# bio-phys/BioEM

Measured on AMD Instinct MI355X. Metric: image-comparisons/sec (orient×CTF×particle) at 224²; log P max-abs-diff vs CPU, higher is better.
Workload: dtype f32

## Files before the change

### bioem_amd/csrc/bioem_hip.hip

```cpp
#define BIOEM_MAIN_TU 1
#include "engine_types.hpp"

#include <rccl/rccl.h>

#include <dlfcn.h>

#include <map>
#include <memory>
#include <mutex>
#include <queue>
#include <string>
#include <vector>

namespace
{

struct HipErr
{
  std::string msg;
};

#define HIP_CHECK(h, expr)                                                                                         \
  do                                                                                                               \
  {                                                                                                                \
// ... 1119 lines not shown
    const int Rl = 2 * P.halfR, off = fastm2_off(Rl, P.gs), nAcc = fastm2_acc(Rl, P.gs);
    const int nS = (P.N1 + 1) / 2;
    twk.assign((size_t) nS * nAcc * 2, make_float2(0.f, 0.f));
    for (int s2 = 0; s2 < nS; s2++)
      for (int ac = 0; ac < nAcc; ac++)
      {
        const long long dx = (long long) (2 * off * (ac / off) + (ac % off) - kFm2WD) * P.gs;
        for (int e = 0; e < 2; e++)
          if (2 * s2 + e < P.N1)
            twk[((size_t) s2 * nAcc + ac) * 2 + e] = twiddle(dx * (2 * s2 + e), N);
      }
    std::vector<float> bt(fastm2_btab_floats(h->H, P.nyq));
    for (size_t K = 0; K < bt.size() / 192; K++)
      for (int ct = 0; ct < 3; ct++)
        for (int l = 0; l < 64; l++)
        {
          const long long ky = 2 * (long long) K + (l >> 5), dy = (long long) (16 * ct + (l & 15) - kFm2WD) * P.gs;
          const float2 w = twiddle(ky * dy, N);
          bt[(K * 3 + ct) * 64 + l] = ((l >> 4) & 1) ? w.y : w.x;
        }
    if (upload(h, h->dBtab, bt.data(), bt.size()))
      return 1;
  }
  if (P.family == KF_FAST || P.family == KF_FASTM || P.family == KF_ROWS || P.family == KF_ODDFFT)
  {
    const int NW = 2 * P.winD + 1;
    const int nK1 = P.family == KF_ROWS ? N : P.N1;
    twk.resize((size_t) nK1 * NW);
    for (int k1 = 0; k1 < nK1; k1++)
      for (int d = -P.winD; d <= P.winD; d++)
        twk[(size_t) k1 * NW + d + P.winD] = twiddle((long long) d * P.gs * k1, N);
  }
  if (!twk.empty() && upload(h, h->dTwk, twk.data(), twk.size()))
    return 1;
  if (P.nyq)
  {
    const int NW = 2 * P.nyqWD + 1, R2 = P.halfR;
    std::vector<float2> twn((size_t) (N / 2) * NW * 2);
    for (int k1 = 0; k1 < P.N1; k1++)
      for (int k2p = 0; k2p < R2; k2p++)
        for (int m = -P.nyqWD; m <= P.nyqWD; m++)
          for (int e = 0; e < 2; e++)
          {
            const long long kx = (long long) P.N1 * (2 * k2p + e) + k1;
            twn[(((size_t) (k1 * R2 + k2p) * NW) + (m + P.nyqWD)) * 2 + e] = twiddle(kx * m * P.gs, N);
          }
    if (upload(h, h->dTwNyq, twn.data(), twn.size()))
      return 1;
  }
  std::vector<float2> tw(N + 1);
  std::vector<double2> twd(N);
  for (int k = 0; k <= N; k++)
    tw[k] = twiddle(k, N);
  for (int k = 0; k < N; k++)
    twd[k] = twiddle_d(k, N);
  std::vector<double2> lt(64);
  for (int i = 0; i < 64; i++)
  {
    const double c = 1.0 / (1.0 + ((double) i + 0.5) / 64.0);
    lt[i] = make_double2(c, -log(c));
  }
  if (upload(h, h->dTw, tw.data(), tw.size()) || upload(h, h->dTwD, twd.data(), twd.size()) ||
      upload(h, h->dDisp, P.disp.data(), P.disp.size()) || upload(h, h->dLtab, lt.data(), lt.size()))
    return 1;
  if (const char *lg = getenv("BIOEM_SIGNATURE_LOG"))
    if (FILE *f = fopen(lg, "a"))
    {
      fprintf(f, "%s\n", bioem_hip_kernel_signature(h));
      if (P.nyq)
        fprintf(f, "k_nyquist_rows<%d, %d>\n", P.nyqWD, h->nMaps <= 64 ? 4 : 1);
      fclose(f);
    }
  return 0;
}

int bioem_hip_create(bioem_hip_handle *out, int device, const bioem_hip_param_device *pd, int nMaps, int nAngles,
                     int nCTF, int algo)
{
  return create_impl(out, device, pd, nMaps, nAngles, nCTF, algo, false, 0, nAngles);
}

int bioem_hip_create_shard(bioem_hip_handle *out, int device, const bioem_hip_param_device *pd, int nMaps, int nAngles,
                           int nCTF, int algo, int iOrientBegin, int iOrientEnd)
{
  return create_impl(out, device, pd, nMaps, nAngles, nCTF, algo, true, iOrientBegin, iOrientEnd);
}

int bioem_hip_destroy(bioem_hip_handle h)
{
  if (!h)
    return 0;
  hipSetDevice(h->device);
  if (h->stream)
    hipStreamSynchronize(h->stream);
  drain_events(h);
  drain_phases(h);
  for (hipEvent_t e : h->evPool)
    hipEventDestroy(e);
  if (h->prepStream)
    hipStreamSynchronize(h->prepStream);
  for (const bioem_hip_ctx::Alloc &al : h->allocs)
    if (al.pinned)
      hipHostFree(al.p);
    else
      hipFree(al.p);
  for (int k = 0; k < 2; k++)
// ... 1130 lines not shown
```

### bioem_amd/csrc/compare_args.hpp

```cpp
#ifndef BIOEM_COMPARE_ARGS_HPP
#define BIOEM_COMPARE_ARGS_HPP

namespace
{

struct CompareArgs
{
  const float2 *ref;
  const float2 *conv;
  const bioem_hip_param5 *params;
  const double2 *postc;
  const float *sumRef, *sumsqRef;
  const float2 *tw;
  const int *disp;
  const double2 *ltab;
  const float2 *twk;
  const float2 *twnyq;
  const float *btab;
  float *tnyq;
  Partial *partials;
  int ldPart;
  int N, H, N1, nd, maxD, nOC, nMaps, algo;
  int Hp;
  int pchunk;
  int gs;
  int ndx, ndy;
  int ts, nyqWD;
  int split;
  PD pd;
};

}

#endif
```

### bioem_amd/csrc/compare_fast.hpp

```cpp
#ifndef BIOEM_COMPARE_FAST_HPP
#define BIOEM_COMPARE_FAST_HPP

namespace
{

typedef const float2 __attribute__((address_space(4))) *const_float2_ptr;
__device__ __forceinline__ const_float2_ptr as_constant(const float2 *p)
{
  return (const_float2_ptr) (unsigned long long) p;
}

template <typename T>
__device__ __forceinline__ T *uniform_ptr(T *p)
{
  const unsigned long long v = (unsigned long long) p;
  const unsigned lo = __builtin_amdgcn_readfirstlane((unsigned) v);
  const unsigned hi = __builtin_amdgcn_readfirstlane((unsigned) (v >> 32));
  return (T *) (((unsigned long long) hi << 32) | lo);
}

__device__ __noinline__ double log_slow_path(float f) { return log((double) f); }

__device__ __forceinline__ double log_of_float(float f, const double2 *ltab)
{
// ... 144 lines not shown
  for (int v = 0; v < B; v++)
  {
    double lp = w.A * lg[v] + w.t2;
    lp -= w.prior;
    lpf[v] = ok[v] ? (float) lp : -INFINITY;
    lpe[v] = (algo == 1) ? (double) lpf[v] : lp;
  }
  float mb = lpf[0], vb = cc[0];
  int ib = ok[0] ? id[0] : 0x7fffffff;
#pragma unroll
  for (int v = 1; v < B; v++)
  {
    const bool t = ok[v] && (lpf[v] > mb || (lpf[v] == mb && id[v] < ib));
    mb = t ? lpf[v] : mb;
    ib = t ? id[v] : ib;
    vb = t ? cc[v] : vb;
  }
  const bool take = mb > L.m || (mb == L.m && ib < L.id);
  const float newm = fmaxf(L.m, mb);
  double sum = (L.m == newm) ? L.s : L.s * exp_fast_nonpos((double) L.m - (double) newm);
#pragma unroll
  for (int v = 0; v < B; v++)
  {
    const double e = exp_fast_nonpos(lpe[v] - (double) newm);
    sum += ok[v] ? e : 0.;
  }
  L.s = sum;
  L.m = newm;
  L.id = take ? ib : L.id;
  L.val = take ? vb : L.val;
}

__device__ __forceinline__ bool fast_block_pair(const CompareArgs &a, int &p, int &ocg)
{
  const int ocGroups = (a.nOC + 3) >> 2;
  if (a.pchunk < 0)
  {
    const int x = blockIdx.x & 7, q = blockIdx.x >> 3;
    ocg = (q / a.nMaps) * 8 + x;
    p = q % a.nMaps;
    return ocg < ocGroups;
  }
  const int per = a.pchunk * ocGroups;
  int c = blockIdx.x / per;
  const int nch = (a.nMaps + a.pchunk - 1) / a.pchunk;
  c = min(c, nch - 1);
  const int rem = blockIdx.x - c * per;
  const int pc = min(a.pchunk, a.nMaps - c * a.pchunk);
  ocg = rem / pc;
  p = c * a.pchunk + (rem - ocg * pc);
  return true;
}

template <int NR, bool STATIC, int NP, int TS>
__device__ __forceinline__ void window_accumulate(const float2 *Tl, const float2 *twl, int N, int step, int idx0,
                                                  const int (&rowoff)[NR], int nr, float (&acc)[NR], int npairs = NP)
{
  int idx = idx0;
#pragma unroll 2
  for (int kp = 0; kp < npairs; kp++)
  {
    const float2 w0 = twl[idx];
    idx += step;
    if (idx >= N)
      idx -= N;
    const float2 w1 = twl[idx];
    idx += step;
    if (idx >= N)
      idx -= N;
#pragma unroll
    for (int r = 0; r < NR; r++)
    {
      if (STATIC || r < nr)
      {
        const float4 t = *reinterpret_cast<const float4 *>(&Tl[(STATIC ? rowoff[0] + r * TS : rowoff[r]) + 2 * kp]);
        float v = acc[r];
        v = fmaf(t.x, w0.x, v);
        v = fmaf(-t.y, w0.y, v);
        v = fmaf(t.z, w1.x, v);
        v = fmaf(-t.w, w1.y, v);
        acc[r] = v;
      }
    }
  }
}

#define FFT_IN(k) (is_pow2(R) ? bitrevR<R>(k) : DIGITREV<R>.pos[k])
#define FFT_OUT(n) (n)
#define FFT_RUN(xr, xi)                                                                                            \
  do                                                                                                               \
  {                                                                                                                \
    if constexpr (is_pow2(R))                                                                                      \
      fft_inverse_dit<R>(xr, xi);                                                                                  \
    else                                                                                                           \
      fft_inverse_mixed<R>(xr, xi);                                                                                \
  } while (0)
template <int WD, int R, bool NYQ, int GS>
__global__ __launch_bounds__(256, 3) void k_compare_fast(const CompareArgs a)
{
  static_assert(WD <= 10, "windows of at most 21 rows; 27 / 31 rows: k_compare_fastm");
  constexpr int NW = 2 * WD + 1;
  constexpr int R2 = R / 2;
  constexpr int RD = (R2 % 4 == 0) ? 4 : (R2 == 15) ? 3 : (R2 % 5 == 0) ? 5 : (R2 % 3 == 0) ? 3 : (R2 % 2 == 0) ? 2 : 1;
  constexpr int NR = (WD <= 5) ? 3 : 7;
  constexpr int TS = 66;
  extern __shared__ __align__(16) unsigned char smem[];
  const int N = a.N, H = a.H, N1 = a.N1;
  float2 *twl = reinterpret_cast<float2 *>(smem);
  int *displ = reinterpret_cast<int *>(smem + (size_t) ((N + 2) & ~1) * 8);
  double2 *ltab = reinterpret_cast<double2 *>(smem + (size_t) ((N + 2) & ~1) * 8 + 256);
  float2 *Tall = reinterpret_cast<float2 *>(smem + (size_t) ((N + 2) & ~1) * 8 + 256 + 1024);
  const int wave = __builtin_amdgcn_readfirstlane((int) (threadIdx.x >> 6));
  const int lane = threadIdx.x & 63;
  float2 *Tl = Tall + (size_t) wave * NW * TS;

  for (int t = threadIdx.x; t <= N; t += blockDim.x)
    twl[t] = a.tw[t];
  int *dinv = displ + 32;
  const int mD = a.maxD / GS;
  for (int t = threadIdx.x; t < a.nd; t += blockDim.x)
  {
    const int dv = a.disp[t];
    displ[t] = dv;
    const int m = dv / GS + mD;
    if (m >= 0 && m < 32)
      dinv[m] = t;
  }
  for (int t = threadIdx.x; t < 64; t += blockDim.x)
    ltab[t] = a.ltab[t];
  __syncthreads();

  int p, ocg;
  if (!fast_block_pair(a, p, ocg))
    return;
  const int oc_raw = ocg * 4 + wave;
  const bool oc_valid = oc_raw < a.nOC;
  const int oc = oc_valid ? oc_raw : a.nOC - 1;
  const int Hp = a.Hp;
  const size_t M = (size_t) N * Hp;
  const auto rsrcF = __builtin_amdgcn_make_buffer_rsrc(uniform_ptr(const_cast<float2 *>(a.ref + (size_t) p * M)), 0,
                                                       (int) (M * sizeof(float2)), 0x00020000);
  const auto rsrcC = __builtin_amdgcn_make_buffer_rsrc(uniform_ptr(const_cast<float2 *>(a.conv + (size_t) oc * M)), 0,
                                                       (int) (M * sizeof(float2)), 0x00020000);

  const int nd = a.nd;
  const int G = 64 / nd;
  const int nr = (nd + G - 1) / G;
  const int iy = lane % nd, grp = lane / nd;
  const bool wactive = grp < G;
  const int dy = displ[iy];
  const int step = dy < 0 ? dy + N : dy;
  const bool is_static = (nr == NR) && (nd == G * NR) && (nd == 2 * mD + 1);
  float acc[NR];
#pragma unroll
  for (int r = 0; r < NR; r++)
    acc[r] = 0.f;
  auto row_of = [&](int r) -> int {
    int ix = wactive ? grp * nr + r : r;
    if (ix >= nd)
      ix = nd - 1;
    return (displ[ix] / GS + WD) * TS;
  };
  const int rowbase = is_static ? ((wactive ? grp : 0) * NR - mD + WD) * TS : row_of(0);

  const int nblk = NYQ ? (H - 1 + 63) / 64 : (H + 63) / 64;
  const unsigned rowbytes = (unsigned) Hp * 16u;
  constexpr bool SPLIT_OK = !(NYQ && R == 32);
  const int sHalf = (N1 + 1) >> 1;
  const int hsel = lane >> 5;
  const unsigned halfoff = (unsigned) (hsel * sHalf * R2) * rowbytes;
  auto lane_offset = [&](int b) -> unsigned {
    const bool sp = SPLIT_OK && a.split && b == nblk - 1;
    const int kyb = b * 64 + (sp ? (lane & 31) : lane);
    return (unsigned) (kyb < H ? kyb : H - 1) * 16u + (sp ? halfoff : 0u);
  };
  u32x4 rf[RD], rc[RD];
  {
    const unsigned lo0 = lane_offset(0);
#pragma unroll
    for (int t = 0; t < RD; t++)
    {
      rf[t] = __builtin_amdgcn_raw_buffer_load_b128(rsrcF, lo0, (unsigned) t * rowbytes, 0);
      rc[t] = __builtin_amdgcn_raw_buffer_load_b128(rsrcC, lo0, (unsigned) t * rowbytes, 0);
    }
  }
  for (int blk = 0; blk < nblk; blk++)
  {
    const bool split = SPLIT_OK && a.split && blk == nblk - 1;
    const int n1 = split ? sHalf : N1;
    const int ttotal = R2 * n1;
    const int ky = blk * 64 + (split ? (lane & 31) : lane);
    const unsigned laneoff = lane_offset(blk);
    const unsigned laneoff_next = lane_offset(min(blk + 1, nblk - 1));
    const bool has_next = blk + 1 < nblk;
    float Tr[NW], Ti[NW];
#pragma unroll
    for (int d = 0; d < NW; d++)
    {
      Tr[d] = 0.f;
      Ti[d] = 0.f;
    }
    if (ky < H)
    for (int k1 = 0; k1 < n1; k1++)
    {
      float xr[R], xi[R];
      float2 wk[NW];
      const float2 *twk = a.twk + (size_t) k1 * NW;
#pragma unroll
      for (int d = 0; d < NW; d++)
        wk[d] = twk[d];
#pragma unroll
      for (int k2p = 0; k2p < R2; k2p++)
      {
        const float4 f = as_float4(rf[k2p % RD]);
        const float4 c = as_float4(rc[k2p % RD]);
        xr[FFT_IN(2 * k2p)] = fmaf(c.x, f.x, c.y * f.y);
        xi[FFT_IN(2 * k2p)] = fmaf(c.y, f.x, -(c.x * f.y));
        xr[FFT_IN(2 * k2p + 1)] = fmaf(c.z, f.z, c.w * f.w);
        xi[FFT_IN(2 * k2p + 1)] = fmaf(c.w, f.z, -(c.z * f.w));
        int tn = k1 * R2 + k2p + RD;
        unsigned vo = laneoff;
        if (k2p + RD >= R2 && tn >= ttotal)
        {
          tn = has_next ? tn - ttotal : ttotal - 1;
          vo = has_next ? laneoff_next : laneoff;
        }
        rf[k2p % RD] = __builtin_amdgcn_raw_buffer_load_b128(rsrcF, vo, (unsigned) tn * rowbytes, 0);
        rc[k2p % RD] = __builtin_amdgcn_raw_buffer_load_b128(rsrcC, vo, (unsigned) tn * rowbytes, 0);
        __builtin_amdgcn_sched_barrier(0);
      }
      FFT_RUN(xr, xi);
#pragma unroll
      for (int d = -WD; d <= WD; d++)
      {
        const int pos = FFT_OUT((((d * GS) % R) + R) % R);
        const float2 w = wk[d + WD];
        float tr = Tr[d + WD], ti = Ti[d + WD];
        tr = fmaf(xr[pos], w.x, tr);
        tr = fmaf(-xi[pos], w.y, tr);
        ti = fmaf(xr[pos], w.y, ti);
        ti = fmaf(xi[pos], w.x, ti);
        Tr[d + WD] = tr;
        Ti[d + WD] = ti;
      }
    }
    if (split)
    {
      const float2 *ws = a.twk + (size_t) sHalf * NW;
#pragma unroll
      for (int d = 0; d < NW; d++)
      {
        const float2 w = ws[d];
        const float wx = hsel ? w.x : 1.f, wy = hsel ? w.y : 0.f;
        const float tr = fmaf(-Ti[d], wy, Tr[d] * wx), ti = fmaf(Ti[d], wx, Tr[d] * wy);
        const u32x2 sr = __builtin_amdgcn_permlane32_swap(__float_as_uint(tr), __float_as_uint(tr), false, false);
        const u32x2 si = __builtin_amdgcn_permlane32_swap(__float_as_uint(ti), __float_as_uint(ti), false, false);
        Tr[d] = __uint_as_float(sr.x) + __uint_as_float(sr.y);
        Ti[d] = __uint_as_float(si.x) + __uint_as_float(si.y);
      }
    }
    float wgt = 2.f;
    if (ky == 0 || (((N & 1) == 0) && ky == N / 2))
      wgt = 1.f;
    if (ky >= H || (split && hsel))
      wgt = 0.f;
    {
      __syncthreads();
#pragma unroll
      for (int d = 0; d < NW; d++)
        Tl[d * TS + lane] = make_float2(Tr[d] * wgt, Ti[d] * wgt);
      __syncthreads();
      const int idx0 = (int) (((long long) (blk * 64) * step) % N);
      const int npairs = min(32, (H - blk * 64 + 1) >> 1);
      if (is_static)
      {
        const int rowoff[NR] = {rowbase};
        window_accumulate<NR, true, 32, TS>(Tl, twl, N, step, idx0, rowoff, nr, acc, npairs);
      }
      else
      {
        int rowoff[NR];
#pragma unroll
        for (int r = 0; r < NR; r++)
          rowoff[r] = row_of(r);
        window_accumulate<NR, false, 32, TS>(Tl, twl, N, step, idx0, rowoff, nr, acc, npairs);
      }
    }
  }
  if (NYQ)
  {
    const float *tq = a.tnyq + ((size_t) p * a.ldPart + oc) * NW;
    const float sg = (dy & 1) ? -1.f : 1.f;
#pragma unroll
    for (int r = 0; r < NR; r++)
      acc[r] = fmaf(sg, tq[is_static ? rowbase / TS + r : row_of(r) / TS], acc[r]);
  }

  const double2 pc = a.postc[oc];
  const PostW pw = post_consts(a.pd.Ntotpi, N, a.params[oc], a.sumRef[p], a.sumsqRef[p], pc.x, pc.y);
  LseF L;
  L.m = -INFINITY;
  L.s = 0.;
  L.id = 0x7fffffff;
  L.val = 0.f;
  {
    constexpr int PB = NR > 8 ? 8 : NR;
#pragma unroll
    for (int r0 = 0; r0 < NR; r0 += PB)
    {
      float accv[PB];
      int idv[PB];
      bool okv[PB];
#pragma unroll
      for (int j = 0; j < PB; j++)
      {
        const int r = r0 + j < NR ? r0 + j : NR - 1;
        const int ixs = grp * nr + r;
        okv[j] = r0 + j < NR && r < nr && wactive && ixs < a.ndx && iy < a.ndy;
        const int ix = is_static ? dinv[min(ixs, 31)] : ixs;
        accv[j] = acc[r];
        idv[j] = ix * nd + iy;
      }
      posterior_batch<PB>(L, accv, idv, okv, pw, ltab, a.algo);
    }
  }
  lsef_wave_reduce(L);
  if (lane == 0 && oc_valid)
  {
    Partial r;
    r.sumExp = L.s;
    r.best = L.m;
    r.id = L.id;
    r.value = L.val;
    r.pad = 0;
    a.partials[(size_t) p * a.ldPart + oc] = r;
  }
}

template <int WD, int Q>
__global__ __launch_bounds__(256) void k_nyquist_rows(const CompareArgs a)
{
  static_assert(Q == 1 || Q == 4, "one thread per pair, or one per pair and wave");
  constexpr int NW = 2 * WD + 1;
  __shared__ float part[Q == 4 ? 2 * 64 * NW : 1];
  const int N = a.N, H = a.H, N1 = a.N1;
  const int R2 = N / (2 * N1);
  const int tilesOC = (a.nOC + 15) / 16;
  const int tp = blockIdx.x / tilesOC, to = blockIdx.x - tp * tilesOC;
  const int q = Q == 1 ? 0 : __builtin_amdgcn_readfirstlane((int) (threadIdx.x >> 6));
  const int t = Q == 1 ? threadIdx.x : threadIdx.x & 63;
  const int p = tp * (16 / Q) + (t >> 4), oc = to * 16 + (t & 15);
  const bool valid = p < a.nMaps && oc < a.nOC;
  const size_t M = (size_t) N * a.Hp;
  const float2 *F = a.ref + (size_t) (valid ? p : 0) * M;
  const float2 *C = a.conv + (size_t) (valid ? oc : 0) * M;
  float acc[NW];
#pragma unroll
  for (int d = 0; d < NW; d++)
    acc[d] = 0.f;
  const int nRP = N1 * R2 / Q;
  constexpr int NB = WD > 31 ? 4 : 8;
  for (int rp0 = q * nRP; rp0 < (q + 1) * nRP; rp0 += NB)
  {
    float4 cb[NB], fb[NB];
#pragma unroll
    for (int u = 0; u < NB; u++)
    {
      const size_t li = ((size_t) (rp0 + u) * a.Hp + N / 2) * 2;
      cb[u] = *reinterpret_cast<const float4 *>(C + li);
      fb[u] = *reinterpret_cast<const float4 *>(F + li);
    }
#pragma unroll
    for (int u = 0; u < NB; u++)
    {
// ... 61 lines not shown
```

### bioem_amd/csrc/compare_fast_own.hpp

```cpp
#ifndef BIOEM_COMPARE_FAST_OWN_HPP
#define BIOEM_COMPARE_FAST_OWN_HPP

namespace
{

typedef int __attribute__((ext_vector_type(4))) own_i32x4;
typedef const own_i32x4 __attribute__((address_space(4))) *const_int4_ptr;

template <int WD, int R, bool NYQ, int GS>
__global__ __launch_bounds__(256, 3) void k_compare_fast_own(const CompareArgs a, const int4 *__restrict__ blocks)
{
  static_assert(WD <= 10, "windows of at most 21 rows; 27 / 31 rows: k_compare_fastm");
  constexpr int NW = 2 * WD + 1;
  constexpr int R2 = R / 2;
  constexpr int RD = (R2 % 4 == 0) ? 4 : (R2 == 15) ? 3 : (R2 % 5 == 0) ? 5 : (R2 % 3 == 0) ? 3 : (R2 % 2 == 0) ? 2 : 1;
  constexpr int NR = (WD <= 5) ? 3 : 7;
  constexpr int TS = 66;
  extern __shared__ __align__(16) unsigned char smem[];
  const int N = a.N, H = a.H, N1 = a.N1;
  float2 *twl = reinterpret_cast<float2 *>(smem);
  int *displ = reinterpret_cast<int *>(smem + (size_t) ((N + 2) & ~1) * 8);
  double2 *ltab = reinterpret_cast<double2 *>(smem + (size_t) ((N + 2) & ~1) * 8 + 256);
  float2 *Tall = reinterpret_cast<float2 *>(smem + (size_t) ((N + 2) & ~1) * 8 + 256 + 1024);
  const int wave = __builtin_amdgcn_readfirstlane((int) (threadIdx.x >> 6));
  const int lane = threadIdx.x & 63;
  float2 *Tl = Tall + (size_t) wave * NW * TS;

  for (int t = threadIdx.x; t <= N; t += blockDim.x)
    twl[t] = a.tw[t];
  int *dinv = displ + 32;
  const int mD = a.maxD / GS;
  for (int t = threadIdx.x; t < a.nd; t += blockDim.x)
  {
    const int dv = a.disp[t];
    displ[t] = dv;
    const int m = dv / GS + mD;
    if (m >= 0 && m < 32)
      dinv[m] = t;
  }
  for (int t = threadIdx.x; t < 64; t += blockDim.x)
    ltab[t] = a.ltab[t];
  __syncthreads();

  const own_i32x4 be = *((const_int4_ptr) (unsigned long long) (blocks + blockIdx.x));
  const int p = be.x;
  const int oc_raw = be.y + wave;
  const bool oc_valid = oc_raw < be.z;
  const int oc = oc_valid ? oc_raw : be.z - 1;
  const int Hp = a.Hp;
  const size_t M = (size_t) N * Hp;
  const auto rsrcF = __builtin_amdgcn_make_buffer_rsrc(uniform_ptr(const_cast<float2 *>(a.ref + (size_t) p * M)), 0,
                                                       (int) (M * sizeof(float2)), 0x00020000);
  const auto rsrcC = __builtin_amdgcn_make_buffer_rsrc(uniform_ptr(const_cast<float2 *>(a.conv + (size_t) oc * M)), 0,
                                                       (int) (M * sizeof(float2)), 0x00020000);

  const int nd = a.nd;
  const int G = 64 / nd;
  const int nr = (nd + G - 1) / G;
  const int iy = lane % nd, grp = lane / nd;
  const bool wactive = grp < G;
  const int dy = displ[iy];
  const int step = dy < 0 ? dy + N : dy;
  const bool is_static = (nr == NR) && (nd == G * NR) && (nd == 2 * mD + 1);
  float acc[NR];
#pragma unroll
  for (int r = 0; r < NR; r++)
    acc[r] = 0.f;
  auto row_of = [&](int r) -> int {
    int ix = wactive ? grp * nr + r : r;
    if (ix >= nd)
      ix = nd - 1;
    return (displ[ix] / GS + WD) * TS;
  };
  const int rowbase = is_static ? ((wactive ? grp : 0) * NR - mD + WD) * TS : row_of(0);

  const int nblk = NYQ ? (H - 1 + 63) / 64 : (H + 63) / 64;
  const unsigned rowbytes = (unsigned) Hp * 16u;
  constexpr bool SPLIT_OK = !(NYQ && R == 32);
  const int sHalf = (N1 + 1) >> 1;
  const int hsel = lane >> 5;
  const unsigned halfoff = (unsigned) (hsel * sHalf * R2) * rowbytes;
  auto lane_offset = [&](int b) -> unsigned {
    const bool sp = SPLIT_OK && a.split && b == nblk - 1;
    const int kyb = b * 64 + (sp ? (lane & 31) : lane);
    return (unsigned) (kyb < H ? kyb : H - 1) * 16u + (sp ? halfoff : 0u);
  };
  u32x4 rf[RD], rc[RD];
  {
    const unsigned lo0 = lane_offset(0);
#pragma unroll
    for (int t = 0; t < RD; t++)
    {
      rf[t] = __builtin_amdgcn_raw_buffer_load_b128(rsrcF, lo0, (unsigned) t * rowbytes, 0);
      rc[t] = __builtin_amdgcn_raw_buffer_load_b128(rsrcC, lo0, (unsigned) t * rowbytes, 0);
    }
  }
  for (int blk = 0; blk < nblk; blk++)
  {
    const bool split = SPLIT_OK && a.split && blk == nblk - 1;
    const int n1 = split ? sHalf : N1;
    const int ttotal = R2 * n1;
    const int ky = blk * 64 + (split ? (lane & 31) : lane);
    const unsigned laneoff = lane_offset(blk);
    const unsigned laneoff_next = lane_offset(min(blk + 1, nblk - 1));
    const bool has_next = blk + 1 < nblk;
    float Tr[NW], Ti[NW];
#pragma unroll
    for (int d = 0; d < NW; d++)
    {
      Tr[d] = 0.f;
      Ti[d] = 0.f;
    }
    if (ky < H)
    for (int k1 = 0; k1 < n1; k1++)
    {
      float xr[R], xi[R];
      float2 wk[NW];
      const float2 *twk = a.twk + (size_t) k1 * NW;
#pragma unroll
      for (int d = 0; d < NW; d++)
        wk[d] = twk[d];
#pragma unroll
      for (int k2p = 0; k2p < R2; k2p++)
      {
        const float4 f = as_float4(rf[k2p % RD]);
        const float4 c = as_float4(rc[k2p % RD]);
        xr[FFT_IN(2 * k2p)] = fmaf(c.x, f.x, c.y * f.y);
        xi[FFT_IN(2 * k2p)] = fmaf(c.y, f.x, -(c.x * f.y));
        xr[FFT_IN(2 * k2p + 1)] = fmaf(c.z, f.z, c.w * f.w);
        xi[FFT_IN(2 * k2p + 1)] = fmaf(c.w, f.z, -(c.z * f.w));
        int tn = k1 * R2 + k2p + RD;
        unsigned vo = laneoff;
        if (k2p + RD >= R2 && tn >= ttotal)
        {
          tn = has_next ? tn - ttotal : ttotal - 1;
          vo = has_next ? laneoff_next : laneoff;
        }
        rf[k2p % RD] = __builtin_amdgcn_raw_buffer_load_b128(rsrcF, vo, (unsigned) tn * rowbytes, 0);
        rc[k2p % RD] = __builtin_amdgcn_raw_buffer_load_b128(rsrcC, vo, (unsigned) tn * rowbytes, 0);
        __builtin_amdgcn_sched_barrier(0);
      }
      FFT_RUN(xr, xi);
#pragma unroll
      for (int d = -WD; d <= WD; d++)
      {
        const int pos = FFT_OUT((((d * GS) % R) + R) % R);
        const float2 w = wk[d + WD];
        float tr = Tr[d + WD], ti = Ti[d + WD];
        tr = fmaf(xr[pos], w.x, tr);
        tr = fmaf(-xi[pos], w.y, tr);
        ti = fmaf(xr[pos], w.y, ti);
        ti = fmaf(xi[pos], w.x, ti);
        Tr[d + WD] = tr;
        Ti[d + WD] = ti;
      }
    }
    if (split)
    {
      const float2 *ws = a.twk + (size_t) sHalf * NW;
#pragma unroll
      for (int d = 0; d < NW; d++)
      {
        const float2 w = ws[d];
        const float wx = hsel ? w.x : 1.f, wy = hsel ? w.y : 0.f;
        const float tr = fmaf(-Ti[d], wy, Tr[d] * wx), ti = fmaf(Ti[d], wx, Tr[d] * wy);
        const u32x2 sr = __builtin_amdgcn_permlane32_swap(__float_as_uint(tr), __float_as_uint(tr), false, false);
        const u32x2 si = __builtin_amdgcn_permlane32_swap(__float_as_uint(ti), __float_as_uint(ti), false, false);
        Tr[d] = __uint_as_float(sr.x) + __uint_as_float(sr.y);
        Ti[d] = __uint_as_float(si.x) + __uint_as_float(si.y);
      }
    }
    float wgt = 2.f;
    if (ky == 0 || (((N & 1) == 0) && ky == N / 2))
      wgt = 1.f;
    if (ky >= H || (split && hsel))
      wgt = 0.f;
    {
      __syncthreads();
#pragma unroll
      for (int d = 0; d < NW; d++)
        Tl[d * TS + lane] = make_float2(Tr[d] * wgt, Ti[d] * wgt);
      __syncthreads();
      const int idx0 = (int) (((long long) (blk * 64) * step) % N);
      const int npairs = min(32, (H - blk * 64 + 1) >> 1);
      if (is_static)
      {
        const int rowoff[NR] = {rowbase};
        window_accumulate<NR, true, 32, TS>(Tl, twl, N, step, idx0, rowoff, nr, acc, npairs);
      }
      else
      {
        int rowoff[NR];
#pragma unroll
        for (int r = 0; r < NR; r++)
          rowoff[r] = row_of(r);
        window_accumulate<NR, false, 32, TS>(Tl, twl, N, step, idx0, rowoff, nr, acc, npairs);
      }
    }
  }
  if (NYQ)
  {
    const float *tq = a.tnyq + (size_t) oc * NW;
    const float sg = (dy & 1) ? -1.f : 1.f;
#pragma unroll
    for (int r = 0; r < NR; r++)
      acc[r] = fmaf(sg, tq[is_static ? rowbase / TS + r : row_of(r) / TS], acc[r]);
  }

  const double2 pc = a.postc[oc];
  const PostW pw = post_consts(a.pd.Ntotpi, N, a.params[oc], a.sumRef[p], a.sumsqRef[p], pc.x, pc.y);
  LseF L;
  L.m = -INFINITY;
  L.s = 0.;
  L.id = 0x7fffffff;
  L.val = 0.f;
  {
    constexpr int PB = NR > 8 ? 8 : NR;
#pragma unroll
    for (int r0 = 0; r0 < NR; r0 += PB)
    {
      float accv[PB];
      int idv[PB];
      bool okv[PB];
#pragma unroll
      for (int j = 0; j < PB; j++)
      {
        const int r = r0 + j < NR ? r0 + j : NR - 1;
        const int ixs = grp * nr + r;
        okv[j] = r0 + j < NR && r < nr && wactive && ixs < a.ndx && iy < a.ndy;
        const int ix = is_static ? dinv[min(ixs, 31)] : ixs;
        accv[j] = acc[r];
        idv[j] = ix * nd + iy;
      }
      posterior_batch<PB>(L, accv, idv, okv, pw, ltab, a.algo);
    }
  }
  lsef_wave_reduce(L);
  if (lane == 0 && oc_valid)
  {
    Partial r;
    r.sumExp = L.s;
    r.best = L.m;
    r.id = L.id;
    r.value = L.val;
    r.pad = 0;
    a.partials[oc] = r;
  }
}

template <int WD>
__global__ __launch_bounds__(256) void k_nyquist_rows_own(const CompareArgs a, const int *__restrict__ slotParticle,
                                                          int row0, int nCTF)
{
  constexpr int NW = 2 * WD + 1;
  __shared__ float part[2 * 64 * NW];
  const int N = a.N, N1 = a.N1;
  const int R2 = N / (2 * N1);
  const int q = __builtin_amdgcn_readfirstlane((int) (threadIdx.x >> 6));
  const int t = threadIdx.x & 63;
  const int oc = blockIdx.x * 64 + t;
  const bool valid = oc < a.nOC;
  const int p = valid ? slotParticle[(row0 + oc) / nCTF] : 0;
  const size_t M = (size_t) N * a.Hp;
  const float2 *F = a.ref + (size_t) p * M;
  const float2 *C = a.conv + (size_t) (valid ? oc : 0) * M;
  float acc[NW];
#pragma unroll
  for (int d = 0; d < NW; d++)
    acc[d] = 0.f;
  const int nRP = N1 * R2 / 4;
  constexpr int NB = 8;
  for (int rp0 = q * nRP; rp0 < (q + 1) * nRP; rp0 += NB)
  {
    float4 cb[NB], fb[NB];
#pragma unroll
    for (int u = 0; u < NB; u++)
    {
      const size_t li = ((size_t) (rp0 + u) * a.Hp + N / 2) * 2;
      cb[u] = *reinterpret_cast<const float4 *>(C + li);
      fb[u] = *reinterpret_cast<const float4 *>(F + li);
    }
#pragma unroll
    for (int u = 0; u < NB; u++)
    {
      const float4 c = cb[u], f = fb[u];
// ... 57 lines not shown
```

### bioem_amd/csrc/kernel_select.hpp

```cpp
#ifndef BIOEM_KERNEL_SELECT_HPP
#define BIOEM_KERNEL_SELECT_HPP

namespace
{

typedef void (*fast_kernel_t)(const CompareArgs);

typedef BioemKernelEntry KernelEntry;

#ifdef BIOEM_SLIM
const KernelEntry kSlimTable[] = {
#ifdef BIOEM_SLIM_FAST
    {KF_FAST, {BIOEM_SLIM_FAST, 0, 0}, reinterpret_cast<const void *>(k_compare_fast<BIOEM_SLIM_FAST>)},
#endif
#ifdef BIOEM_SLIM_FASTM
    {KF_FASTM, {BIOEM_SLIM_FASTM, 0, 0}, reinterpret_cast<const void *>(k_compare_fastm<BIOEM_SLIM_FASTM>)},
#endif
#ifdef BIOEM_SLIM_FASTM2
    {KF_FASTM2, {BIOEM_SLIM_FASTM2, 0, 0, 0}, reinterpret_cast<const void *>(k_compare_fastm2<BIOEM_SLIM_FASTM2>)},
#endif
#ifdef BIOEM_SLIM_W2
    {KF_WIDE2, {BIOEM_SLIM_W2}, reinterpret_cast<const void *>(k_compare_wide2<BIOEM_SLIM_W2>)},
#endif
    {KF_GENERIC, {0, 0, 0, 0, 0, 0}, reinterpret_cast<const void *>(k_compare_generic)}};
// ... 11 lines not shown
#else
  switch (family)
  {
  case KF_FAST: tabs[nt] = bioem_kernels_fast(&cnt[nt]); nt++; break;
  case KF_FASTM: tabs[nt] = bioem_kernels_fastm(&cnt[nt]); nt++; break;
  case KF_FASTM2: tabs[nt] = bioem_kernels_fastm2(&cnt[nt]); nt++; break;
  case KF_WIDE2:
    tabs[nt] = bioem_kernels_wide2_short(&cnt[nt]); nt++;
    tabs[nt] = bioem_kernels_wide2_16(&cnt[nt]); nt++;
    tabs[nt] = bioem_kernels_wide2_long(&cnt[nt]); nt++;
    break;
  default: tabs[nt] = bioem_kernels_odd(&cnt[nt]); nt++; break;
  }
#endif
  for (int t = 0; t < nt; t++)
    for (int i = 0; i < cnt[t]; i++)
    {
      const KernelEntry &e = tabs[t][i];
      if (e.fn && e.family == family && e.a[0] == a0 && e.a[1] == a1 && e.a[2] == a2 && e.a[3] == a3 && e.a[4] == a4 &&
          e.a[5] == a5)
        return reinterpret_cast<fast_kernel_t>(const_cast<void *>(e.fn));
    }
  return nullptr;
}

typedef void (*own_kernel_t)(const CompareArgs, const int4 *);
typedef void (*nyq_own_kernel_t)(const CompareArgs, const int *, int, int);

own_kernel_t find_own_kernel(int family, int wd, int R, bool nyq, int gs)
{
#ifdef BIOEM_SLIM
  return nullptr;
#else
  if (family != KF_FAST || (nyq && !bioem_nyquist_rows_own(wd)))
    return nullptr;
  int n = 0;
  const KernelEntry *tab = bioem_kernels_fast_own(&n);
  for (int i = 0; i < n; i++)
  {
    const KernelEntry &e = tab[i];
    if (e.fn && e.family == KF_FAST && e.a[0] == wd && e.a[1] == R && e.a[2] == (int) nyq && e.a[3] == gs)
      return reinterpret_cast<own_kernel_t>(const_cast<void *>(e.fn));
  }
  return nullptr;
#endif
}

size_t compare_lds_bytes(int N, int H, int NW, int waves, int rows = 0)
{
  const int Hs = (H + 1) & ~1;
  const size_t dispBytes = ((size_t) NW * 4 + 255) & ~(size_t) 255;
  return (size_t) ((N + 2) & ~1) * 8 + dispBytes + (size_t) waves * (rows ? rows : NW) * Hs * 8;
}
size_t fast_lds_bytes(int N, int NW, int waves)
{
  return (size_t) ((N + 2) & ~1) * 8 + 256 + 1024 + (size_t) waves * NW * 66 * 8;
}
size_t fastm_lds_bytes(int N)
{
  return (size_t) 2 * fastm_table_floats(N) * 4 + 128 + 1024 + (size_t) 4 * 2 * 32 * 33 * 4 + (size_t) 4 * 16 * 64 * 4;
}
size_t fastm2_lds_bytes()
{
  return (size_t) 256 + 1024 + (size_t) 4 * kFm2WaveFloats * 4 + 256;
}
size_t wide2_lds_bytes(int N, int R, int rows2, int ts, int nw = 4)
{
  const size_t slots = (size_t) nw * R * 64 * 8, tblock = (size_t) rows2 * ts * 8;
  return (size_t) ((N + 2) & ~1) * 8 + 512 + 1024 + 256 + std::max(slots, tblock);
}
constexpr size_t kLdsCU = 160 * 1024;

struct KernelPlan
{
  std::vector<int> disp;
  int nd = 0, gs = 1, winD = 0;
  int family = KF_GENERIC;
  int halfR = 0, N1 = 0;
  int oddR = 0;
  bool nyq = false;
  int nyqWD = 0;
  int tileT = 0, tilesPerAxis = 1;
  std::vector<int> tileCenter, tileValid;
  int w2NRW = 0, w2NBLK = 0, w2TS = 0, w2Rows2 = 0, w2Halves = 1, w2NW = 4;
  int genericWaves = 4;
  int genericRows = 0;
  size_t ldsBytes = 0;
  fast_kernel_t fn = nullptr;
  const char *err = nullptr;
};

void fft_lengths(int N, int cap, bool allowMixed, std::vector<int> &out)
{
  int p2 = 2;
  for (int r : {32, 16, 8, 4})
    if (r <= cap && N % r == 0)
    {
      p2 = r;
      break;
    }
  if (allowMixed && p2 < 8)
    for (int r : {30, 20, 18, 12, 10, 6})
      if (r <= cap && N % r == 0 && r > p2)
        out.push_back(r);
  out.push_back(p2);
  for (int r : {16, 8, 4, 2})
    if (r < p2 && N % r == 0)
      out.push_back(r);
}
// ... 119 lines not shown
      P.nyq = nyq;
      P.w2NBLK = nblk;
      P.w2NRW = r.nrw;
      P.w2NW = r.nw;
      P.w2Halves = halves;
      P.w2TS = ts;
      P.w2Rows2 = halves == 2 ? hrows : rows2;
      P.nyqWD = mD <= 20 ? 20 : mD <= 31 ? 31 : 42;
      P.ldsBytes = wide2_lds_bytes(N, R, P.w2Rows2, ts, r.nw);
      return true;
    }
  }
  return false;
}

bool take_window(KernelPlan &P, int family, fast_kernel_t fn, int N, int R, bool nyq, int wd, size_t ldsBytes)
{
  P.family = family;
  P.fn = fn;
  P.halfR = R / 2;
  P.N1 = N / R;
  P.nyq = nyq;
  P.nyqWD = nyq ? wd : 0;
  P.winD = wd;
  P.ldsBytes = ldsBytes;
  return true;
}

bool plan_window_kernel(KernelPlan &P, int N, int H, int winD, bool untiled)
{
  const bool nyq = N % 2 == 0 && (N / 2) % 64 == 0;
  if (N % 2 == 0 && N >= 8)
  {
    if (winD > 10)
    {
      std::vector<int> lens;
      if (nyq)
        lens.push_back(16);
      else
        fft_lengths(N, 16, P.gs == 1, lens);
      for (int R : lens)
      {
        if (const fast_kernel_t fn = find_kernel(KF_FASTM, winD, R, nyq, P.gs))
          return take_window(P, KF_FASTM, fn, N, R, nyq, winD, fastm_lds_bytes(N));
      }
      return false;
    }
    const bool nyq32 = !nyq && (N / 2) % 64 == 32 && (N <= 256 || (N == 320 && winD == 10)) &&
                       !getenv("BIOEM_NO_SPLIT_LAST");
    if (nyq32)
    {
      const int R = winD == 5 ? 8 : 16;
      if (const fast_kernel_t fn = find_kernel(KF_FAST, winD, R, true, P.gs))
        return take_window(P, KF_FAST, fn, N, R, true, winD, fast_lds_bytes(N, 2 * winD + 1, 4));
    }
    std::vector<int> lens;
    if (nyq)
    {
      lens.push_back(32);
      if (winD != 5)
        lens.push_back(16);
      else if (N <= 160)
        lens.push_back(8);
    }
    else
      fft_lengths(N, 32, P.gs == 1, lens);
    {
      if (N <= 256)
      {
        static const int pref21[] = {16, 12, 20, 18, 10, 32, 30, 8, 6, 4, 2};
        static const int pref11s[] = {8, 16, 12, 10, 18, 20, 32, 30, 6, 4, 2};
        static const int pref11l[] = {16, 12, 18, 10, 8, 20, 32, 30, 6, 4, 2};
        const int *pref = winD == 5 ? (N <= 160 ? pref11s : pref11l) : pref21;
        auto rank = [&](int r) {
          for (int k = 0; k < 11; k++)
            if (pref[k] == r)
              return k;
          return 11;
        };
        std::stable_sort(lens.begin(), lens.end(), [&](int a, int b) { return rank(a) < rank(b); });
      }
    }
    for (int R : lens)
    {
      int wd = winD;
      const int nblkF = nyq ? (H - 1) / 64 : (H + 63) / 64;
      if (wd == 5 && untiled && ((nblkF >= 4 && R <= 16) || N / R >= 40) &&
          find_kernel(KF_FAST, 10, R, nyq, P.gs))
        wd = 10;
      if (const fast_kernel_t fn = find_kernel(KF_FAST, wd, R, nyq, P.gs))
        return take_window(P, KF_FAST, fn, N, R, nyq, wd, fast_lds_bytes(N, 2 * wd + 1, 4));
    }
    return false;
  }
  if (N >= 8)
  {
    if (P.gs == 1)
      for (int r : {25, 15, 9, 5, 3})
        if (N % r == 0)
          if (const fast_kernel_t fn = find_kernel(KF_ODDFFT, winD, r))
          {
            P.family = KF_ODDFFT;
            P.oddR = r;
            P.N1 = N / r;
            P.fn = fn;
            P.winD = winD;
            P.ldsBytes = fast_lds_bytes(N, 2 * winD + 1, 4);
            return true;
          }
    if (const fast_kernel_t fn = find_kernel(KF_ROWS, winD, P.gs))
    {
      P.family = KF_ROWS;
      P.fn = fn;
      P.winD = winD;
      P.ldsBytes = fast_lds_bytes(N, 2 * winD + 1, 4);
      return true;
    }
  }
  return false;
}

KernelPlan plan_kernels(int N, int maxD, int grid, int algo)
{
  KernelPlan P;
  const int H = N / 2 + 1;
  if (algo == 1)
  {
    for (int c = 0; c <= maxD; c += grid)
      P.disp.push_back(c);
    for (int c = N - maxD; c < N; c += grid)
      P.disp.push_back(c - N);
  }
  else
  {
    const int NxDisp = 2 * (maxD / grid) + 1;
    for (int m = 0; m < NxDisp; m++)
      P.disp.push_back(m * grid - maxD);
  }
  P.nd = (int) P.disp.size();
  {
    int gg = 0;
    for (int d : P.disp)
    {
      int x = d < 0 ? -d : d, y = gg;
// ... 134 lines not shown
```

Baseline: 50.84 million.

## Exploit ±m displacement symmetry in 21-row window accumulation with precomputed twiddle slices

For window half-width 10 with FFT length up to 18, the fast compare kernel now pairs displacements +m and -m. It accumulates the real and imaginary products separately and forms both correlations from their sum and difference, using a per-block precomputed twiddle slice that is streamed into LDS. This removes the per-row strided twiddle index walk and halves the multiply work across symmetric displacements. In exchange it relayouts lanes (3 lanes per row, 8 accumulators), prefetches table slices from global memory each block, and makes the host-side table larger.

```diff
diff --git a/bioem_amd/csrc/bioem_hip.hip b/bioem_amd/csrc/bioem_hip.hip
--- a/bioem_amd/csrc/bioem_hip.hip
+++ b/bioem_amd/csrc/bioem_hip.hip
@@ -1195,6 +1195,15 @@
   std::vector<double2> twd(N);
   for (int k = 0; k <= N; k++)
     tw[k] = twiddle(k, N);
+  if (P.family == KF_FAST && sym_window_ok(P.winD, 2 * P.halfR, P.nyq, P.gs))
+  {
+    const size_t nPairs = (size_t) ((h->H + 63) / 64) * 32;
+    tw.resize(sym_table_offset(N) + nPairs * kSymEntries * 2, make_float2(0.f, 0.f));
+    for (size_t kp = 0; kp < nPairs; kp++)
+      for (int j = 0; j <= 10; j++)
+        for (int e = 0; e < 2; e++)
+          tw[sym_table_offset(N) + (kp * kSymEntries + j) * 2 + e] = twiddle((long long) (2 * kp + e) * j * P.gs, N);
+  }
   for (int k = 0; k < N; k++)
     twd[k] = twiddle_d(k, N);
   std::vector<double2> lt(64);
diff --git a/bioem_amd/csrc/compare_args.hpp b/bioem_amd/csrc/compare_args.hpp
--- a/bioem_amd/csrc/compare_args.hpp
+++ b/bioem_amd/csrc/compare_args.hpp
@@ -30,6 +30,17 @@
   PD pd;
 };
 
+constexpr int kSymEntries = 12;
+constexpr int kSymSliceFloat2 = 32 * kSymEntries * 2;
+constexpr int kSymSliceBytes = kSymSliceFloat2 * 8;
+constexpr bool sym_window_ok(int WD, int R, bool NYQ, int GS) { return WD == 10 && R <= 18; }
+__host__ __device__ constexpr int sym_table_offset(int N) { return (N + 2) & ~1; }
+__host__ __device__ constexpr size_t fast_head_bytes(int N, bool sym)
+{
+  const size_t twBytes = (size_t) ((N + 2) & ~1) * 8;
+  return sym && twBytes < (size_t) kSymSliceBytes ? (size_t) kSymSliceBytes : twBytes;
+}
+
 }
 
 #endif
diff --git a/bioem_amd/csrc/compare_fast.hpp b/bioem_amd/csrc/compare_fast.hpp
--- a/bioem_amd/csrc/compare_fast.hpp
+++ b/bioem_amd/csrc/compare_fast.hpp
@@ -220,10 +220,11 @@
   return true;
 }
 
-template <int NR, bool STATIC, int NP, int TS>
+template <int NR, bool STATIC, int NP, int TS, int NA>
 __device__ __forceinline__ void window_accumulate(const float2 *Tl, const float2 *twl, int N, int step, int idx0,
-                                                  const int (&rowoff)[NR], int nr, float (&acc)[NR], int npairs = NP)
-{
+                                                  const int (&rowoff)[NR], int nr, float (&acc)[NA], int npairs = NP)
+{
+  static_assert(NA >= NR, "one accumulator per row of the lane");
   int idx = idx0;
 #pragma unroll 2
   for (int kp = 0; kp < npairs; kp++)
@@ -249,6 +250,28 @@
         v = fmaf(-t.w, w1.y, v);
         acc[r] = v;
       }
+    }
+  }
+}
+
+template <int TS>
+__device__ __forceinline__ void window_accumulate_sym(const float2 *Trow, const float4 *tab, float (&acc)[8], int npairs)
+{
+#pragma unroll 2
+  for (int kp = 0; kp < npairs; kp++)
+  {
+    const float4 t = *reinterpret_cast<const float4 *>(&Trow[2 * kp]);
+#pragma unroll
+    for (int j = 0; j < 4; j++)
+    {
+      const float4 w = tab[kp * kSymEntries + j];
+      float va = acc[j], vb = acc[4 + j];
+      va = fmaf(t.x, w.x, va);
+      vb = fmaf(t.y, w.y, vb);
+      va = fmaf(t.z, w.z, va);
+      vb = fmaf(t.w, w.w, vb);
+      acc[j] = va;
+      acc[4 + j] = vb;
     }
   }
 }
@@ -272,20 +295,25 @@
   constexpr int RD = (R2 % 4 == 0) ? 4 : (R2 == 15) ? 3 : (R2 % 5 == 0) ? 5 : (R2 % 3 == 0) ? 3 : (R2 % 2 == 0) ? 2 : 1;
   constexpr int NR = (WD <= 5) ? 3 : 7;
   constexpr int TS = 66;
+  constexpr bool SYM = sym_window_ok(WD, R, NYQ, GS);
+  constexpr int NA = SYM ? 8 : NR;
   extern __shared__ __align__(16) unsigned char smem[];
   const int N = a.N, H = a.H, N1 = a.N1;
+  const size_t headBytes = fast_head_bytes(N, SYM);
   float2 *twl = reinterpret_cast<float2 *>(smem);
-  int *displ = reinterpret_cast<int *>(smem + (size_t) ((N + 2) & ~1) * 8);
-  double2 *ltab = reinterpret_cast<double2 *>(smem + (size_t) ((N + 2) & ~1) * 8 + 256);
-  float2 *Tall = reinterpret_cast<float2 *>(smem + (size_t) ((N + 2) & ~1) * 8 + 256 + 1024);
+  int *displ = reinterpret_cast<int *>(smem + headBytes);
+  double2 *ltab = reinterpret_cast<double2 *>(smem + headBytes + 256);
+  float2 *Tall = reinterpret_cast<float2 *>(smem + headBytes + 256 + 1024);
   const int wave = __builtin_amdgcn_readfirstlane((int) (threadIdx.x >> 6));
   const int lane = threadIdx.x & 63;
   float2 *Tl = Tall + (size_t) wave * NW * TS;
 
-  for (int t = threadIdx.x; t <= N; t += blockDim.x)
-    twl[t] = a.tw[t];
   int *dinv = displ + 32;
   const int mD = a.maxD / GS;
+  const bool symw = SYM && a.nd == NW && mD == WD;
+  if (!symw)
+    for (int t = threadIdx.x; t <= N; t += blockDim.x)
+      twl[t] = a.tw[t];
   for (int t = threadIdx.x; t < a.nd; t += blockDim.x)
   {
     const int dv = a.disp[t];
@@ -319,10 +347,14 @@
   const int dy = displ[iy];
   const int step = dy < 0 ? dy + N : dy;
   const bool is_static = (nr == NR) && (nd == G * NR) && (nd == 2 * mD + 1);
-  float acc[NR];
-#pragma unroll
-  for (int r = 0; r < NR; r++)
+  float acc[NA];
+#pragma unroll
+  for (int r = 0; r < NA; r++)
     acc[r] = 0.f;
+  const int srow = min(lane / 3, NW - 1), sgrp = lane % 3;
+  const float2 *Trow = Tl + srow * TS;
+  const float4 *stab = reinterpret_cast<const float4 *>(smem) + sgrp * 4;
+  const float2 *symsrc = a.tw + sym_table_offset(N) + threadIdx.x;
   auto row_of = [&](int r) -> int {
     int ix = wactive ? grp * nr + r : r;
     if (ix >= nd)
@@ -367,6 +399,13 @@
     {
       Tr[d] = 0.f;
       Ti[d] = 0.f;
+    }
+    float2 tabv[3] = {};
+    if (symw)
+    {
+#pragma unroll
+      for (int u = 0; u < 3; u++)
+        tabv[u] = symsrc[blk * kSymSliceFloat2 + u * 256];
     }
     if (ky < H)
     for (int k1 = 0; k1 < n1; k1++)
@@ -437,10 +476,21 @@
 #pragma unroll
       for (int d = 0; d < NW; d++)
         Tl[d * TS + lane] = make_float2(Tr[d] * wgt, Ti[d] * wgt);
+      if (symw)
+      {
+#pragma unroll
+        for (int u = 0; u < 3; u++)
+          twl[u * 256 + threadIdx.x] = tabv[u];
+      }
       __syncthreads();
       const int idx0 = (int) (((long long) (blk * 64) * step) % N);
       const int npairs = min(32, (H - blk * 64 + 1) >> 1);
-      if (is_static)
+      if (symw)
+      {
+        if constexpr (SYM)
+          window_accumulate_sym<TS>(Trow, stab, acc, npairs);
+      }
+      else if (!SYM && is_static)
       {
         const int rowoff[NR] = {rowbase};
         window_accumulate<NR, true, 32, TS>(Tl, twl, N, step, idx0, rowoff, nr, acc, npairs);
@@ -459,9 +509,21 @@
   {
     const float *tq = a.tnyq + ((size_t) p * a.ldPart + oc) * NW;
     const float sg = (dy & 1) ? -1.f : 1.f;
-#pragma unroll
-    for (int r = 0; r < NR; r++)
-      acc[r] = fmaf(sg, tq[is_static ? rowbase / TS + r : row_of(r) / TS], acc[r]);
+    if (symw)
+    {
+      if constexpr (SYM)
+      {
+#pragma unroll
+        for (int j = 0; j < 4; j++)
+          acc[j] = fmaf((((sgrp * 4 + j) * GS) & 1) ? -1.f : 1.f, tq[srow], acc[j]);
+      }
+    }
+    else
+    {
+#pragma unroll
+      for (int r = 0; r < NR; r++)
+        acc[r] = fmaf(sg, tq[is_static ? rowbase / TS + r : row_of(r) / TS], acc[r]);
+    }
   }
 
   const double2 pc = a.postc[oc];
@@ -472,22 +534,41 @@
   L.id = 0x7fffffff;
   L.val = 0.f;
   {
-    constexpr int PB = NR > 8 ? 8 : NR;
-#pragma unroll
-    for (int r0 = 0; r0 < NR; r0 += PB)
+    constexpr int PB = NA > 8 ? 8 : NA;
+#pragma unroll
+    for (int r0 = 0; r0 < NA; r0 += PB)
     {
       float accv[PB];
       int idv[PB];
       bool okv[PB];
-#pragma unroll
-      for (int j = 0; j < PB; j++)
-      {
-        const int r = r0 + j < NR ? r0 + j : NR - 1;
-        const int ixs = grp * nr + r;
-        okv[j] = r0 + j < NR && r < nr && wactive && ixs < a.ndx && iy < a.ndy;
-        const int ix = is_static ? dinv[min(ixs, 31)] : ixs;
-        accv[j] = acc[r];
-        idv[j] = ix * nd + iy;
+      if (symw)
+      {
+        if constexpr (SYM)
+        {
+          const int ixv = dinv[srow];
+#pragma unroll
+          for (int j = 0; j < 8; j++)
+          {
+            const int q = j >> 1, m = sgrp * 4 + q;
+            const int iyv = dinv[min(max((j & 1) ? mD - m : mD + m, 0), 31)];
+            okv[j] = lane < 3 * NW && m <= WD && !((j & 1) && m == 0) && srow < a.ndx && iyv < a.ndy;
+            accv[j] = (j & 1) ? acc[q] + acc[4 + q] : acc[q] - acc[4 + q];
+            idv[j] = ixv * nd + iyv;
+          }
+        }
+      }
+      else
+      {
+#pragma unroll
+        for (int j = 0; j < PB; j++)
+        {
+          const int r = r0 + j < NR ? r0 + j : NR - 1;
+          const int ixs = grp * nr + r;
+          okv[j] = r0 + j < NR && r < nr && wactive && ixs < a.ndx && iy < a.ndy;
+          const int ix = is_static ? dinv[min(ixs, 31)] : ixs;
+          accv[j] = acc[r];
+          idv[j] = ix * nd + iy;
+        }
       }
       posterior_batch<PB>(L, accv, idv, okv, pw, ltab, a.algo);
     }
diff --git a/bioem_amd/csrc/compare_fast_own.hpp b/bioem_amd/csrc/compare_fast_own.hpp
--- a/bioem_amd/csrc/compare_fast_own.hpp
+++ b/bioem_amd/csrc/compare_fast_own.hpp
@@ -16,20 +16,25 @@
   constexpr int RD = (R2 % 4 == 0) ? 4 : (R2 == 15) ? 3 : (R2 % 5 == 0) ? 5 : (R2 % 3 == 0) ? 3 : (R2 % 2 == 0) ? 2 : 1;
   constexpr int NR = (WD <= 5) ? 3 : 7;
   constexpr int TS = 66;
+  constexpr bool SYM = sym_window_ok(WD, R, NYQ, GS);
+  constexpr int NA = SYM ? 8 : NR;
   extern __shared__ __align__(16) unsigned char smem[];
   const int N = a.N, H = a.H, N1 = a.N1;
+  const size_t headBytes = fast_head_bytes(N, SYM);
   float2 *twl = reinterpret_cast<float2 *>(smem);
-  int *displ = reinterpret_cast<int *>(smem + (size_t) ((N + 2) & ~1) * 8);
-  double2 *ltab = reinterpret_cast<double2 *>(smem + (size_t) ((N + 2) & ~1) * 8 + 256);
-  float2 *Tall = reinterpret_cast<float2 *>(smem + (size_t) ((N + 2) & ~1) * 8 + 256 + 1024);
+  int *displ = reinterpret_cast<int *>(smem + headBytes);
+  double2 *ltab = reinterpret_cast<double2 *>(smem + headBytes + 256);
+  float2 *Tall = reinterpret_cast<float2 *>(smem + headBytes + 256 + 1024);
   const int wave = __builtin_amdgcn_readfirstlane((int) (threadIdx.x >> 6));
   const int lane = threadIdx.x & 63;
   float2 *Tl = Tall + (size_t) wave * NW * TS;
 
-  for (int t = threadIdx.x; t <= N; t += blockDim.x)
-    twl[t] = a.tw[t];
   int *dinv = displ + 32;
   const int mD = a.maxD / GS;
+  const bool symw = SYM && a.nd == NW && mD == WD;
+  if (!symw)
+    for (int t = threadIdx.x; t <= N; t += blockDim.x)
+      twl[t] = a.tw[t];
   for (int t = threadIdx.x; t < a.nd; t += blockDim.x)
   {
     const int dv = a.disp[t];
@@ -62,10 +67,14 @@
   const int dy = displ[iy];
   const int step = dy < 0 ? dy + N : dy;
   const bool is_static = (nr == NR) && (nd == G * NR) && (nd == 2 * mD + 1);
-  float acc[NR];
-#pragma unroll
-  for (int r = 0; r < NR; r++)
+  float acc[NA];
+#pragma unroll
+  for (int r = 0; r < NA; r++)
     acc[r] = 0.f;
+  const int srow = min(lane / 3, NW - 1), sgrp = lane % 3;
+  const float2 *Trow = Tl + srow * TS;
+  const float4 *stab = reinterpret_cast<const float4 *>(smem) + sgrp * 4;
+  const float2 *symsrc = a.tw + sym_table_offset(N) + threadIdx.x;
   auto row_of = [&](int r) -> int {
     int ix = wactive ? grp * nr + r : r;
     if (ix >= nd)
@@ -110,6 +119,13 @@
     {
       Tr[d] = 0.f;
       Ti[d] = 0.f;
+    }
+    float2 tabv[3] = {};
+    if (symw)
+    {
+#pragma unroll
+      for (int u = 0; u < 3; u++)
+        tabv[u] = symsrc[blk * kSymSliceFloat2 + u * 256];
     }
     if (ky < H)
     for (int k1 = 0; k1 < n1; k1++)
@@ -180,10 +196,21 @@
 #pragma unroll
       for (int d = 0; d < NW; d++)
         Tl[d * TS + lane] = make_float2(Tr[d] * wgt, Ti[d] * wgt);
+      if (symw)
+      {
+#pragma unroll
+        for (int u = 0; u < 3; u++)
+          twl[u * 256 + threadIdx.x] = tabv[u];
+      }
       __syncthreads();
       const int idx0 = (int) (((long long) (blk * 64) * step) % N);
       const int npairs = min(32, (H - blk * 64 + 1) >> 1);
-      if (is_static)
+      if (symw)
+      {
+        if constexpr (SYM)
+          window_accumulate_sym<TS>(Trow, stab, acc, npairs);
+      }
+      else if (!SYM && is_static)
       {
         const int rowoff[NR] = {rowbase};
         window_accumulate<NR, true, 32, TS>(Tl, twl, N, step, idx0, rowoff, nr, acc, npairs);
@@ -202,9 +229,21 @@
   {
     const float *tq = a.tnyq + (size_t) oc * NW;
     const float sg = (dy & 1) ? -1.f : 1.f;
-#pragma unroll
-    for (int r = 0; r < NR; r++)
-      acc[r] = fmaf(sg, tq[is_static ? rowbase / TS + r : row_of(r) / TS], acc[r]);
+    if (symw)
+    {
+      if constexpr (SYM)
+      {
+#pragma unroll
+        for (int j = 0; j < 4; j++)
+          acc[j] = fmaf((((sgrp * 4 + j) * GS) & 1) ? -1.f : 1.f, tq[srow], acc[j]);
+      }
+    }
+    else
+    {
+#pragma unroll
+      for (int r = 0; r < NR; r++)
+        acc[r] = fmaf(sg, tq[is_static ? rowbase / TS + r : row_of(r) / TS], acc[r]);
+    }
   }
 
   const double2 pc = a.postc[oc];
@@ -215,22 +254,41 @@
   L.id = 0x7fffffff;
   L.val = 0.f;
   {
-    constexpr int PB = NR > 8 ? 8 : NR;
-#pragma unroll
-    for (int r0 = 0; r0 < NR; r0 += PB)
+    constexpr int PB = NA > 8 ? 8 : NA;
+#pragma unroll
+    for (int r0 = 0; r0 < NA; r0 += PB)
     {
       float accv[PB];
       int idv[PB];
       bool okv[PB];
-#pragma unroll
-      for (int j = 0; j < PB; j++)
-      {
-        const int r = r0 + j < NR ? r0 + j : NR - 1;
-        const int ixs = grp * nr + r;
-        okv[j] = r0 + j < NR && r < nr && wactive && ixs < a.ndx && iy < a.ndy;
-        const int ix = is_static ? dinv[min(ixs, 31)] : ixs;
-        accv[j] = acc[r];
-        idv[j] = ix * nd + iy;
+      if (symw)
+      {
+        if constexpr (SYM)
+        {
+          const int ixv = dinv[srow];
+#pragma unroll
+          for (int j = 0; j < 8; j++)
+          {
+            const int q = j >> 1, m = sgrp * 4 + q;
+            const int iyv = dinv[min(max((j & 1) ? mD - m : mD + m, 0), 31)];
+            okv[j] = lane < 3 * NW && m <= WD && !((j & 1) && m == 0) && srow < a.ndx && iyv < a.ndy;
+            accv[j] = (j & 1) ? acc[q] + acc[4 + q] : acc[q] - acc[4 + q];
+            idv[j] = ixv * nd + iyv;
+          }
+        }
+      }
+      else
+      {
+#pragma unroll
+        for (int j = 0; j < PB; j++)
+        {
+          const int r = r0 + j < NR ? r0 + j : NR - 1;
+          const int ixs = grp * nr + r;
+          okv[j] = r0 + j < NR && r < nr && wactive && ixs < a.ndx && iy < a.ndy;
+          const int ix = is_static ? dinv[min(ixs, 31)] : ixs;
+          accv[j] = acc[r];
+          idv[j] = ix * nd + iy;
+        }
       }
       posterior_batch<PB>(L, accv, idv, okv, pw, ltab, a.algo);
     }
diff --git a/bioem_amd/csrc/kernel_select.hpp b/bioem_amd/csrc/kernel_select.hpp
--- a/bioem_amd/csrc/kernel_select.hpp
+++ b/bioem_amd/csrc/kernel_select.hpp
@@ -87,9 +87,9 @@
   const size_t dispBytes = ((size_t) NW * 4 + 255) & ~(size_t) 255;
   return (size_t) ((N + 2) & ~1) * 8 + dispBytes + (size_t) waves * (rows ? rows : NW) * Hs * 8;
 }
-size_t fast_lds_bytes(int N, int NW, int waves)
-{
-  return (size_t) ((N + 2) & ~1) * 8 + 256 + 1024 + (size_t) waves * NW * 66 * 8;
+size_t fast_lds_bytes(int N, int NW, int waves, bool sym = false)
+{
+  return fast_head_bytes(N, sym) + 256 + 1024 + (size_t) waves * NW * 66 * 8;
 }
 size_t fastm_lds_bytes(int N)
 {
@@ -315,7 +315,8 @@
     {
       const int R = winD == 5 ? 8 : 16;
       if (const fast_kernel_t fn = find_kernel(KF_FAST, winD, R, true, P.gs))
-        return take_window(P, KF_FAST, fn, N, R, true, winD, fast_lds_bytes(N, 2 * winD + 1, 4));
+        return take_window(P, KF_FAST, fn, N, R, true, winD,
+                           fast_lds_bytes(N, 2 * winD + 1, 4, sym_window_ok(winD, R, true, P.gs)));
     }
     std::vector<int> lens;
     if (nyq)
@@ -352,7 +353,7 @@
           find_kernel(KF_FAST, 10, R, nyq, P.gs))
         wd = 10;
       if (const fast_kernel_t fn = find_kernel(KF_FAST, wd, R, nyq, P.gs))
-        return take_window(P, KF_FAST, fn, N, R, nyq, wd, fast_lds_bytes(N, 2 * wd + 1, 4));
+        return take_window(P, KF_FAST, fn, N, R, nyq, wd, fast_lds_bytes(N, 2 * wd + 1, 4, sym_window_ok(wd, R, nyq, P.gs)));
     }
     return false;
   }
```

Result: faster. 53.93 million, median of 6 (+6.1%).
